# arturxe2/T-DEED

Hardware: AMD Instinct MI355X
Metric: clips/sec (L=100, 224^2, bf16) forward, per-frame logits (higher is better)
Workload: dtype bf16; 1 GPU; rny002_b8: rny002_gsf + ed_sgp_mixer n_layers=2 ks=7, L=100, 224x224, batch 8/GPU, inference forward, random-init weights; clips_per_gpu=8, parallelism=dp1 (clip-sharded, no collective), hip_graph=True, batches_in_flight=3, sub_batches_per_batch=1, dist_backend=none, dist_ranks=1, self_launched=False

## Files before the change

### include/tdeed_hip.h

```cpp
#ifndef TDEED_HIP_H
#define TDEED_HIP_H
#include <stdint.h>
#ifdef __cplusplus
extern "C" {
#endif

enum { TDEED_F32 = 0, TDEED_BF16 = 1 };
enum { TDEED_ACT_NONE = 0, TDEED_ACT_RELU = 1, TDEED_ACT_GELU = 2 };
enum { TDEED_OK = 0, TDEED_ERR_ARG = -1, TDEED_ERR_LAUNCH = -2, TDEED_ERR_RUNTIME = -3 };

const char* tdeed_last_error(void);
int tdeed_abi_version(void);
int tdeed_device_info(int dev, char* name64, int* n_cu, int* is_gfx950);

int tdeed_stem_fwd(const void* frames , int frames_f32,
                   int N, int H, int W, int crop_top, int crop_left,
                   int crop_h, int crop_w, int flip ,
                   const unsigned char* flip_mask ,
                   const float* w ,
                   const float* scale , const float* shift , void* out,
                   int relu , int dtype, void* stream);

int tdeed_stem_mfma_parts(int crop_h, int crop_w);
int tdeed_stem_mfma_fwd(const void* frames, int frames_f32, int N, int H, int W, int crop_top, int crop_left, int crop_h,
// ... 43 lines not shown
int tdeed_gemm_splitk_fwd(const void* A, long lda, int M, int K, int N, const void* W, long ldw, const float* scale,
                          const float* shift, const void* R, long ldr, int act, void* C, long ldc,
                          float* workspace, void* stream);

int tdeed_se_gate_mfma_fits(int C, int R);
int tdeed_se_gate_mfma_fwd(const float* pooled, int n_parts, float inv_cnt, int N, int C, int R, const void* w1f,
                           const float* b1, const void* w2f, const float* b2, float* gate, void* stream);

int tdeed_gemm_rs_fits(int M, int K, int N);
int tdeed_gemm_rs_fwd(const void* A, long lda, const void* A0, long lda0, int k0, const float* a_scale, int a_scale_rows,
                      int M, int K, int N, const void* Wfrag, const float* scale, const float* shift, const void* R, long ldr,
                      int act, void* C, long ldc, void* C2, long ldc2, int n2, void* stream);

int tdeed_gemm_rs_grid(int M);
int tdeed_gemm_rs_stats_fwd(const void* A, long lda, const void* A0, long lda0, int k0, int M, int K, int N, const void* Wfrag,
                            void* C, long ldc, float* colpart, void* stream);

int tdeed_c1_gconv_set_debug(void* buf);
int tdeed_c1_gconv_fits(int Hi, int Wi, int Cin, int C, int stride);
int tdeed_c1_gconv_slab_tiles(int Hi, int Wi, int C, int stride);
int tdeed_c1_gconv_fwd(const void* x, const void* G, int Fp, int N, int Hi, int Wi, int Cin, int C, int gw, int stride,
                       const void* w1f, const float* s1, const float* h1, const void* wfrag, const float* scale,
                       const float* shift, void* y, float* pooled, void* stream);

int tdeed_bneck_fits(int h, int w, int C, int R);
int tdeed_bneck_set_debug(void* buf);
int tdeed_bneck_fwd(const void* x, const void* G, int Fp, int N, int h, int w, int C, const void* w1f, const float* s1,
                    const float* h1, const void* w2f, const float* s2, const float* h2, const void* se_w1f,
                    const float* se_b1, const void* se_w2f, const float* se_b2, int R, const void* w3f, const float* s3,
                    const float* h3, void* out, void* out2, int n2,
                    int w2_tap_major ,
                    void* stream);
int tdeed_bneck_qtail_fits(int h, int w, int C, int F);
int tdeed_bneck_gs_fwd(const void* x, const void* gx, int ldx, const float* gate, const float* ysum, const float* xsum,
                       const float* cw1, const float* cb1, const float* cw2, const float* cb2, int T, int F, int Fp, int N,
                       int h, int w, int C, const void* w1f, const float* s1, const float* h1, const void* w2f,
                       const float* s2, const float* h2, const void* se_w1f, const float* se_b1, const void* se_w2f,
                       const float* se_b2, int R, const void* w3f, const float* s3, const float* h3, void* out, void* out2,
                       int n2, int w2_tap_major, const void* q_wqf, const float* q_bn, int q_F, float* Q, void* stream);


int tdeed_se_gate_fwd(const float* pooled, int n_parts, float inv_cnt, int N, int C, int R,
                      const float* w1t, const float* b1, const float* w2t, const float* b2,
                      float* gate, void* stream);

int tdeed_se_gate_bf16_fwd(const float* pooled, int n_parts, float inv_cnt, int N, int C, int R,
// ... 278 lines not shown
```

### t-deed_amd/_lib.py

```python
import ctypes
import os
from ctypes import c_int, c_long, c_float, c_double, c_void_p, c_char_p, c_uint64, POINTER

import torch

CSRC = os.path.join(os.path.dirname(os.path.abspath(__file__)), "csrc")
LIB_PATH = os.path.join(CSRC, "libtdeed_hip.so")

F32, BF16 = 0, 1
ACT_NONE, ACT_RELU, ACT_GELU = 0, 1, 2


class HipLibraryMissing(RuntimeError):
    pass


class HipCallError(RuntimeError):
    pass


P = c_void_p
_SIGS = {
    "tdeed_abi_version": ([], c_int),
    "tdeed_device_info": ([c_int, c_char_p, POINTER(c_int), POINTER(c_int)], c_int),
# ... 15 lines not shown
    "tdeed_gemm_ws_fits": ([c_int, c_int, c_int], c_int),
    "tdeed_gemm_ws_fwd": ([P, c_long, P, c_long, c_int, P, c_int, c_int, c_int, c_int, P, P, P, P, c_long,
                           c_int, P, c_long, c_int, c_int, c_int, c_int, c_int, P, c_long, c_int, c_int, P], c_int),
    "tdeed_gemm_ws_sc_fits": ([c_int, c_int, c_int, c_int], c_int),
    "tdeed_gemm_ws_sc_fwd": ([P, c_long, P, c_long, c_int, P, c_int, c_int, c_int, c_int, P, P, P, P, c_long, c_int, P, P, P,
                              c_int, P, c_long, c_int, c_int, c_int, c_int, c_int, P, c_long, c_int, c_int, P], c_int),
    "tdeed_gconv3x3_parts": ([c_int, c_int, c_int, c_int, c_int], c_int),
    "tdeed_gconv3x3_mfma_fits": ([c_int, c_int, c_int, c_int], c_int),
    "tdeed_gconv3x3_fwd": ([P, c_int, c_int, c_int, c_int, c_int, c_int, P, P, P, P, P, P, P, P, P, c_int, c_int, P], c_int),
    "tdeed_gemm_splitk_splits": ([c_int], c_int),
    "tdeed_gemm_splitk_fwd": ([P, c_long, c_int, c_int, c_int, P, c_long, P, P, P, c_long, c_int, P, c_long, P, P], c_int),
    "tdeed_se_gate_mfma_fits": ([c_int, c_int], c_int),
    "tdeed_se_gate_mfma_fwd": ([P, c_int, c_float, c_int, c_int, c_int, P, P, P, P, P, P], c_int),
    "tdeed_gemm_rs_fits": ([c_int, c_int, c_int], c_int),
    "tdeed_gemm_rs_grid": ([c_int], c_int),
    "tdeed_gemm_rs_stats_fwd": ([P, c_long, P, c_long, c_int, c_int, c_int, c_int, P, P, c_long, P, P], c_int),
    "tdeed_gemm_rs_fwd": ([P, c_long, P, c_long, c_int, P, c_int, c_int, c_int, c_int, P, P, P, P, c_long, c_int, P, c_long, P,
                           c_long, c_int, P], c_int),
    "tdeed_c1_gconv_set_debug": ([P], c_int),
    "tdeed_c1_gconv_fits": ([c_int, c_int, c_int, c_int, c_int], c_int),
    "tdeed_c1_gconv_slab_tiles": ([c_int, c_int, c_int, c_int], c_int),
    "tdeed_c1_gconv_fwd": ([P, P, c_int, c_int, c_int, c_int, c_int, c_int, c_int, c_int, P, P, P, P, P, P, P, P,
                            P], c_int),
    "tdeed_bneck_fits": ([c_int, c_int, c_int, c_int], c_int),
    "tdeed_bneck_set_debug": ([P], c_int),
    "tdeed_bneck_fwd": ([P, P, c_int, c_int, c_int, c_int, c_int, P, P, P, P, P, P, P, P, P, P, c_int, P, P, P, P, P, c_int,
                         c_int, P], c_int),
    "tdeed_bneck_gs_fwd": ([P, P, c_int, P, P, P, P, P, P, P, c_int, c_int, c_int, c_int, c_int, c_int, c_int, P, P, P, P, P, P, P,
                            P, P, P, c_int, P, P, P, P, P, c_int, c_int, P, P, c_int, P, P], c_int),
    "tdeed_bneck_qtail_fits": ([c_int, c_int, c_int, c_int], c_int),
    "tdeed_gsf_gate_sums_fwd": ([P, c_int, c_int, c_int, c_int, c_int, c_int, P, P, P, P, P, P], c_int),
    "tdeed_bn_slabs": ([c_long], c_int),
    "tdeed_bn_train_stats": ([P, c_long, c_int, P, P, c_float, c_float, P, P, P, P, P, P, P, c_int, P], c_int),
    "tdeed_bn_apply": ([P, c_long, c_int, P, P, P, c_int, P, c_int, P], c_int),
    "tdeed_bn_apply_slice": ([P, c_long, c_int, P, P, P, P, P, c_int, P, P, c_int, c_int, c_int, P], c_int),
    "tdeed_bn_apply2": ([P, c_long, c_int, P, P, P, P, P, c_int, P, c_int, P], c_int),
    "tdeed_bn_train_bwd": ([P, P, P, c_int, c_long, c_int, P, P, P, P, P, P, P, P, P, P, P, c_int, P], c_int),
    "tdeed_fold_rows": ([P, c_long, c_int, c_int, c_int, P, c_long, P], c_int),
    "tdeed_bn_finalize": ([P, P, c_long, c_int, c_long, c_int, P, P, c_float, c_float, P, P, P, P, P, P, P], c_int),
    "tdeed_pool_rows": ([P, P, c_int, c_int, c_int, P, P, c_int, P, c_int, P], c_int),
    "tdeed_se_train_fwd": ([P, c_int, c_int, c_int, P, P, P, P, P, P, P], c_int),
    "tdeed_se_train_bwd": ([P, P, P, c_int, c_int, c_int, P, P, P, P, P, P], c_int),
    "tdeed_scale_rows": ([P, P, P, c_float, c_int, c_int, c_int, P, P, P, c_int, P], c_int),
    "tdeed_gconv3x3_dgrad_stats": ([P, c_int, c_int, c_int, c_int, c_int, P, P, P, P, P, P, P, P, P, P, P], c_int),
    "tdeed_gconv3x3_bwd_stats_bands": ([c_int], c_int),
    "tdeed_gconv3x3_bwd_stats_fits": ([c_int, c_int, c_int, c_int, c_int], c_int),
# ... 211 lines not shown
```

### t-deed_amd/csrc/conv.hip

```cpp
#include "common.h"

template <typename T, typename IN>
__global__ __launch_bounds__(256) void stem_kernel(const IN* __restrict__ frames, int H, int W,
                                                   int top, int left, int ch, int cw, int flip_all,
                                                   const unsigned char* __restrict__ flip_mask,
                                                   const float* __restrict__ w,
                                                   const float* __restrict__ scale,
                                                   const float* __restrict__ shift, T* __restrict__ out,
                                                   int Ho, int Wo, int relu) {
  __shared__ float tile[3][33][34];
  const int n = blockIdx.z;
  const int oy0 = blockIdx.y * 16, ox0 = blockIdx.x * 16;
  const int iy0 = oy0 * 2 - 1, ix0 = ox0 * 2 - 1;
  const float mean[3] = {0.485f, 0.456f, 0.406f};
  const float stdv[3] = {0.229f, 0.224f, 0.225f};
  const IN* src = frames + (long)n * 3 * H * W;
  const int flip = flip_mask ? (int)flip_mask[n] : flip_all;
  for (int i = threadIdx.x; i < 3 * 33 * 33; i += 256) {
    int c = i / (33 * 33);
    int r = i - c * 33 * 33;
    int y = r / 33, x = r - y * 33;
    int iy = iy0 + y, ix = ix0 + x;
    float v = 0.f;
    if (iy >= 0 && iy < ch && ix >= 0 && ix < cw) {
// ... 504 lines not shown
    TD_ISSUE_FENCE();
#pragma unroll
    for (int b8 = 0; b8 < 8; ++b8) {
      const int i = i0 + b8 * 256;
      if (i < total) {
        int j, pix;
        dcpp.divmod(i, pix, j);
        if constexpr (AFF) {
          const bf16x8 t8 = *reinterpret_cast<const bf16x8*>(&v[b8]);
          bf16x8 o8;
#pragma unroll
          for (int e = 0; e < 8; ++e) o8[e] = (bf16_t)fmaxf(fmaf((float)t8[e], ia[e], ib[e]), 0.f);
          v[b8] = *reinterpret_cast<const u32x4*>(&o8);
        }
        *reinterpret_cast<u32x4*>(tile + (long)pix * PS + j * 16) = ok[b8] ? v[b8] : (u32x4){0u, 0u, 0u, 0u};
      }
    }
  }
  __syncthreads();
  gconv_band_mma<STRIDE>(gw_, tile, red, redq, Wi, C, wfrag, scale, shift, y, pooled, pooled_sq, Ho, Wo, nbands, CSP, PS, relu, n, bnd,
                         slab, oy0, nrows_out, bst);
}

template <int STRIDE, int KS1>
__global__ __launch_bounds__(256, KS1 == 4 ? 3 : 1) void c1_gconv_mfma_kernel(const bf16_t* __restrict__ x, const bf16_t* __restrict__ G, int Fp,
                                                            int Hi, int Wi, int Cin, int C, const bf16x8* __restrict__ w1f,
                                                            const float* __restrict__ s1, const float* __restrict__ h1,
                                                            const bf16x8* __restrict__ wfrag, const float* __restrict__ scale,
                                                            const float* __restrict__ shift, bf16_t* __restrict__ y,
                                                            float* __restrict__ pooled, int Ho, int Wo, int band, int nbands,
                                                            int CSP, int PS, int rows_in, int relu, long long* dbg) {
  extern __shared__ __attribute__((aligned(16))) unsigned char tile[];
  __shared__ float red[4][32];
  __shared__ float redq[4][32];
  GC_STAMP(0);
  const long lid = xcd_logical_id(blockIdx.x, gridDim.x);
  const int nslabs_ = (C + CSP - 1) >> (CSP == 64 ? 6 : (CSP == 32 ? 5 : 4));
  int slab, bnd, n, t_;
  td_split(lid, nslabs_, t_, slab);
  td_split(t_, nbands, n, bnd);
  const int oy0 = bnd * band;
  const int nrows_out = min(band, Ho - oy0);
  const int WP = Wi + 2;
  const int iy0 = oy0 * STRIDE - 1;
  const int nrow_used = (nrows_out - 1) * STRIDE + 3;
  const int tid = threadIdx.x, lane = tid & 63, wv = __builtin_amdgcn_readfirstlane(tid >> 6);
  const int pl = lane & 15, q = lane >> 4;
  const int nts = CSP >> 4;
  GcW gw_;
  if constexpr (KS1 <= 2) gw_ = gconv_load_w(wfrag, slab, CSP);
  bf16x8 w1r[4][KS1];
  float a1[4][4], b1[4][4];
#pragma unroll
  for (int t = 0; t < 4; ++t) {
    const int tt = slab * nts + min(t, nts - 1);
#pragma unroll
    for (int ks = 0; ks < KS1; ++ks) w1r[t][ks] = w1f[((long)tt * KS1 + ks) * 64 + lane];
    const int c4 = slab * CSP + t * 16 + 4 * q;
    const bool ok = t < nts && c4 < C;
    const int cc4 = min(c4, C - 4);
    const f32x4 av = *reinterpret_cast<const f32x4*>(s1 + cc4), bv = *reinterpret_cast<const f32x4*>(h1 + cc4);
#pragma unroll
    for (int e = 0; e < 4; ++e) {
      a1[t][e] = ok ? av[e] : 0.f;
      b1[t][e] = ok ? bv[e] : 0.f;
    }
  }
  {
    const int cpp = PS >> 4;
    for (int i = tid; i < nrow_used * 2 * cpp; i += 256) {
      const int j = i % cpp, rc = i / cpp;
      const int rr = rc >> 1, col = (rc & 1) ? (Wi + 1) : 0;
      *reinterpret_cast<u32x4*>(tile + ((long)rr * WP + col) * PS + j * 16) = (u32x4){0u, 0u, 0u, 0u};
// ... 39 lines not shown
#pragma unroll
            for (int ks = 0; ks < KS1; ++ks) acc = __builtin_amdgcn_mfma_f32_16x16x32_bf16(w1r[t][ks], xfi[ks], acc, 0, 0, 0);
            if (pok_) {
              bf16x4 o;
#pragma unroll
              for (int e = 0; e < 4; ++e) o[e] = (bf16_t)fmaxf(acc[e] * a1[t][e] + b1[t][e], 0.f);
              *reinterpret_cast<bf16x4*>(dst + t * 32) = o;
            }
          }
        }
      };
      bf16x8 xa[KS1], xb[KS1];
      int ra, ca, rb, cb;
      bool pa = tile_px(wv, ra, ca), pb;
      tile_load(ra, ca, xa);
      for (int tb = wv; tb < ntl; tb += 8) {
        pb = tile_px(tb + 4, rb, cb);
        tile_load(rb, cb, xb);
        tile_mma(pa, ra, ca, xa);
        pa = tile_px(tb + 8, ra, ca);
        tile_load(ra, ca, xa);
        tile_mma(pb, rb, cb, xb);
      }
    } else
    for (int tb = wv; tb < ntl; tb += 4 * NPF) {
      bf16x8 xf[NPF][KS1];
      int rrs[NPF], ccs[NPF];
      bool poks[NPF];
#pragma unroll
      for (int g = 0; g < NPF; ++g) {
        const int t0 = tb + 4 * g;
        const int p = t0 * 16 + pl;
        poks[g] = t0 < ntl && p < npx;
        dwi.divmod(poks[g] ? p : 0, rrs[g], ccs[g]);
        const long pix = (long)(r_lo + rrs[g]) * Wi + ccs[g];
#pragma unroll
        for (int ks = 0; ks < KS1; ++ks) {
          const int k = 32 * ks + 8 * q;
          const bool ok = poks[g] && k < Cin;
          const bf16_t* src = (gn && k < Fp) ? gn + pix * Fp + k : xn + pix * Cin + k;
          const u32x4 v = *reinterpret_cast<const u32x4*>(ok ? src : xn);
          const u32x4 z = {0u, 0u, 0u, 0u};
          const u32x4 w = ok ? v : z;
          xf[g][ks] = *reinterpret_cast<const bf16x8*>(&w);
        }
      }
#pragma unroll
      for (int g = 0; g < NPF; ++g) {
        if (tb + 4 * g >= ntl) break;
        const bool pok = poks[g];
        unsigned char* dst = tile + ((long)(r_lo + rrs[g] - iy0) * WP + ccs[g] + 1) * PS + 8 * q;
#pragma unroll
        for (int t = 0; t < 4; ++t) {
          if (t < nts) {
            f32x4 acc = {0.f, 0.f, 0.f, 0.f};
#pragma unroll
            for (int ks = 0; ks < KS1; ++ks) acc = __builtin_amdgcn_mfma_f32_16x16x32_bf16(w1r[t][ks], xf[g][ks], acc, 0, 0, 0);
            if (pok) {
              bf16x4 o;
#pragma unroll
              for (int e = 0; e < 4; ++e) o[e] = (bf16_t)fmaxf(acc[e] * a1[t][e] + b1[t][e], 0.f);
              *reinterpret_cast<bf16x4*>(dst + t * 32) = o;
            }
          }
        }
      }
    }
  }
  GC_STAMP(2);
  if constexpr (KS1 > 2) gw_ = gconv_load_w(wfrag, slab, CSP);
  __syncthreads();
  GC_STAMP(3);
  gconv_band_mma<STRIDE>(gw_, tile, red, redq, Wi, C, wfrag, scale, shift, y, pooled, nullptr, Ho, Wo, nbands, CSP, PS, relu, n, bnd,
                         slab, oy0, nrows_out, GcStat{nullptr, nullptr, nullptr, nullptr}, dbg);
}

static long long* g_c1g_dbg = nullptr;
extern "C" int tdeed_c1_gconv_set_debug(void* buf) { g_c1g_dbg = (long long*)buf; return TDEED_OK; }

extern "C" int tdeed_gconv3x3_mfma_fits(int Hi, int Wi, int C, int stride) {
  return gc_geom(Hi, Wi, C, stride).band > 0 ? 1 : 0;
}

extern "C" int tdeed_gconv3x3_parts(int Hi, int Wi, int C, int stride, int dtype) {
  if (dtype != TDEED_BF16) return 1;
  GcGeom g = gc_geom(Hi, Wi, C, stride);
  return g.band > 0 ? g.nbands : 1;
}

static int gconv3x3_launch(const void* x, int N, int Hi, int Wi, int C, int gw, int stride, const float* w, const void* wfrag,
                           const float* scale, const float* shift, void* y, float* pooled, float* pooled_sq, const float* in_a,
                           const float* in_b, int relu, int dtype, void* stream, const GcStat bst);
extern "C" int tdeed_gconv3x3_fwd(const void* x, int N, int Hi, int Wi, int C, int gw, int stride,
// ... 59 lines not shown
}
extern "C" int tdeed_c1_gconv_slab_tiles(int Hi, int Wi, int C, int stride) {
  const GcGeom g = gc_geom(Hi, Wi, C, stride);
  return g.nslabs * (g.CSP >> 4);
}
extern "C" int tdeed_c1_gconv_fwd(const void* x, const void* G, int Fp, int N, int Hi, int Wi, int Cin, int C, int gw,
                                  int stride, const void* w1f, const float* s1, const float* h1, const void* wfrag,
                                  const float* scale, const float* shift, void* y, float* pooled, void* stream) {
  TD_CHECK(x && w1f && s1 && h1 && wfrag && scale && shift && y && pooled, "c1_gconv: null pointer");
  TD_CHECK((gw == 8 || gw == 16) && C % gw == 0, "c1_gconv: group width %d / C %d unsupported", gw, C);
  TD_CHECK(stride == 1 || stride == 2, "c1_gconv: stride %d", stride);
  TD_CHECK(N > 0 && N <= 65535 && tdeed_c1_gconv_fits(Hi, Wi, Cin, C, stride), "c1_gconv: Hi=%d Wi=%d Cin=%d C=%d unsupported",
           Hi, Wi, Cin, C);
  TD_CHECK(!G || (Fp % 8 == 0 && Fp > 0 && Fp <= Cin), "c1_gconv: bad splice width %d", Fp);
  const GcGeom g = gc_geom(Hi, Wi, C, stride);
  const int Ho = (Hi - 1) / stride + 1, Wo = (Wi - 1) / stride + 1;
  dim3 grid((unsigned)((long)g.nbands * g.nslabs * N));
  const size_t smem = (size_t)g.rows_in * (Wi + 2) * g.PS;
  hipStream_t st = (hipStream_t)stream;
  const int KS1 = (Cin + 31) / 32;
#define TD_C1G(Sv, Kv)                                                                                                     \
  hipLaunchKernelGGL((c1_gconv_mfma_kernel<Sv, Kv>), grid, dim3(256), smem, st, (const bf16_t*)x, (const bf16_t*)G,           \
                     G ? Fp : 0, Hi, Wi, Cin, C, (const bf16x8*)w1f, s1, h1, (const bf16x8*)wfrag, scale, shift, (bf16_t*)y,  \
                     pooled, Ho, Wo, g.band, g.nbands, g.CSP, g.PS, g.rows_in, 1, g_c1g_dbg)
#define TD_C1G_K(Sv)                                                                                                       \
  do {                                                                                                                     \
    if (KS1 == 1) TD_C1G(Sv, 1); else if (KS1 == 2) TD_C1G(Sv, 2); else if (KS1 == 4) TD_C1G(Sv, 4);                      \
    else TD_C1G(Sv, 5);                                                                                                    \
  } while (0)
  if (stride == 2) TD_C1G_K(2); else TD_C1G_K(1);
#undef TD_C1G_K
#undef TD_C1G
  TD_LAUNCH_CHECK("c1_gconv");
  return TDEED_OK;
}

#define SE_FPB 4
__global__ __launch_bounds__(256) void se_gate_kernel(const float* __restrict__ pooled, int n_parts, float inv_cnt,
                                                      int N, int C, int R, const float* __restrict__ w1t,
                                                      const float* __restrict__ b1,
                                                      const float* __restrict__ w2t,
                                                      const float* __restrict__ b2, float* __restrict__ gate) {
  extern __shared__ float sm[];
  float* sp = sm;
  float* shid = sm + SE_FPB * C;
  const int f0 = blockIdx.x * SE_FPB;
  for (int i = threadIdx.x; i < SE_FPB * C; i += 256) {
    const int f = i / C, c = i - f * C;
    float v = 0.f;
    if (f0 + f < N) {
      const float* src = pooled + ((long)(f0 + f) * n_parts) * C + c;
      for (int q = 0; q < n_parts; ++q) v += src[(long)q * C];
    }
    sp[i] = v * inv_cnt;
  }
  __syncthreads();
// ... 508 lines not shown
```

### t-deed_amd/engine.py

```python
import os
from collections import namedtuple
from types import SimpleNamespace

import numpy as np
import torch

from . import ops, _lib
from .streams import new_stream
from .regnet_spec import regnet_spec, sgp_up_size, pyramid_lengths, first_site_block
from .packing import (_np, _f32, _dense, pack_ws_weights, pack_se_bf16, pack_mfma_frags, pack_se_mfma,
                      pack_front_weights, _stem_frags_np, gs_source_order_columns, _gsf_q_frags_np, pack_gsf_q_frags,
                      _gsf_p_frags_np, pack_gsf_p_frags, pack_gconv_frags, _gconv_frags_np, stem_frags_on_device,
                      gsf_q_frags_on_device, gconv_frag_index, gconv_frags_on_device)

BN_EPS = 1e-5


class _Pool:

    def __init__(self, device):
        self.device = device
        self.free = []
        self.all = []

# ... 114 lines not shown
    o.up = _np(sd[pre + ".convkw1.weight"]).shape[-1]
    o.w_cat = _dense(_np(sd[pre + ".concat_fc.weight"]).reshape(C, 6 * C), act_dtype, device)
    o.b_cat = _f32(_np(sd[pre + ".concat_fc.bias"]), device)
    o.wcg = (pack_mfma_frags(_np(sd[pre + ".concat_fc.weight"]).reshape(C, 6 * C), device, ks_mult=12)
             if act_dtype == torch.bfloat16 and str(device) != "cpu" and C % 16 == 0 and SGP_GEMM else None)
    _pack_mlp(sd, pre, C, o, act_dtype, device)
    return o


def _se(pooled, inv_cnt, bw, gate):
    if bw.se_mf is not None:
        return ops.se_gate_mfma(pooled, inv_cnt, bw.se_mf.w1f, bw.se_b1, bw.se_mf.w2f, bw.se_b2, bw.spec.se_rd, out=gate)
    if bw.se_bf is not None:
        return ops.se_gate_bf16(pooled, inv_cnt, bw.se_bf.se_w1p, bw.se_b1, bw.se_bf.se_w2p, bw.se_b2, bw.spec.se_rd, out=gate)
    return ops.se_gate(pooled, inv_cnt, bw.se_w1t, bw.se_b1, bw.se_w2t, bw.se_b2, out=gate)


BNECK_ONE_LAUNCH = os.environ.get("TDEED_BNECK", "1") == "1"
BNECK_BLEND = True
BNECK_QTAIL = True
C1_GCONV = os.environ.get("TDEED_C1_GCONV", "1") == "1"
C1_GCONV_MAX_CIN = 160
SC_IN_CONV3 = True


BlockForm = namedtuple("BlockForm", "h w h2 w2 one_launch c1g site Fp slice_in q_given blend_in qtail slice_next sc_in_conv3")


def block_forms(blocks, h, w, act_dtype, taps, last_out_is_slice):
    forms = []
    for bi, bw in enumerate(blocks):
        blk = bw.spec
        nbw = blocks[bi + 1] if bi + 1 < len(blocks) else None
        one_launch = bool(BNECK_ONE_LAUNCH and getattr(bw, "fused", None) is not None and bw.se_mf is not None
                          and blk.stride == 1 and not blk.has_downsample and blk.cin == blk.cout
                          and not (last_out_is_slice and nbw is None) and ops.bneck_fits(h, w, blk.cout, blk.se_rd))
        c1g = bool(C1_GCONV and not one_launch and act_dtype == torch.bfloat16 and bw.w2frag is not None
                   and blk.cin <= C1_GCONV_MAX_CIN and ops.c1_gconv_fits(h, w, blk.cin, blk.cout, blk.stride))
        site = blk.gsf_fold > 0
        Fp = (blk.gsf_fold + 7) // 8 * 8 if site else 0
        blend_in = bool(site and one_launch and BNECK_BLEND and bw.gs_src and bw.gs_cw1 is not None and h * w >= 14
                        and 2 * Fp <= blk.cin and ("_features." + blk.name + ".gs_out") not in taps)
        slice_next = (nbw.spec.gsf_fold + 7) // 8 * 8 if (nbw is not None and nbw.spec.gsf_fold) else 0
        qtail = bool(blend_in and BNECK_QTAIL and slice_next and getattr(nbw, "gs_wqf", None) is not None
                     and ops.bneck_qtail_fits(h, w, blk.cout, nbw.spec.gsf_fold))
        sc_in_conv3 = bool(SC_IN_CONV3 and blk.has_downsample and act_dtype == torch.bfloat16 and bw.w3.ws and bw.wd.ws
                           and ops.gemm_ws_sc_fits(blk.cout, blk.cin, blk.cout, act_dtype))
        h2, w2 = (h - 1) // blk.stride + 1, (w - 1) // blk.stride + 1
        slice_in, q_given = bool(site and forms and forms[-1].slice_next == Fp), bool(forms and forms[-1].qtail)
        forms.append(BlockForm(h, w, h2, w2, one_launch, c1g, site, Fp, slice_in, q_given, blend_in, qtail, slice_next, sc_in_conv3))
        h, w = h2, w2
    return forms


class Step:
    __slots__ = ("name", "kernel", "fn", "bytes", "flops")

    def __init__(self, name, kernel, fn, nbytes=0, flops=0):
        self.name, self.kernel, self.fn, self.bytes, self.flops = name, kernel, fn, int(nbytes), int(flops)


def _esz(dt):
    return 2 if dt == torch.bfloat16 else 4


def gemm_cost(M, K, N, es, residual=False, extra=0):
    return (M * K + N * K + M * N * (2 if residual else 1)) * es + extra, 2 * M * K * N


class SgpBuilder:

    def __init__(self, pool, steps, keep, taps, B, act_dtype):
        self.pool, self.steps, self.keep, self.taps, self.B, self.dt = pool, steps, keep, taps, B, act_dtype
# ... 413 lines not shown
        o2 = xs_next.view(-1, f.slice_next) if f.slice_next else None
        q_next = None
        if f.blend_in:
            qt = None
            if f.qtail:
                q_next = pool.take((N, f.h, f.w, 6), torch.float32)
                qt = (nbw.gs_wpf, nbw.gs_bnq, nbw.spec.gsf_fold, q_next)
            run = lambda: ops.bneck_gs(
                x, xg, gb["gate"], gb["ysum"], gb["xsum"], bw.gs_cw1, bw.gs_cb1, bw.gs_cw2, bw.gs_cb2, T, blk.gsf_fold, f.Fp,
                bw.fused.w1f, bw.s1, bw.h1, bw.fused.w2f, bw.s2, bw.h2, bw.se_mf.w1f, bw.se_b1, bw.se_mf.w2f, bw.se_b2,
                blk.se_rd, bw.fused.w3f, bw.s3, bw.h3, out=out, out2=o2, w2_tap_major=bw.fused.w2_tap_major, qtail=qt)
        else:
            G = gb.get("out")
            run = lambda: ops.bneck(
                x, bw.fused.w1f, bw.s1, bw.h1, bw.fused.w2f, bw.s2, bw.h2, bw.se_mf.w1f, bw.se_b1, bw.se_mf.w2f, bw.se_b2,
                blk.se_rd, bw.fused.w3f, bw.s3, bw.h3, G=G, out=out, out2=o2, w2_tap_major=bw.fused.w2_tap_major)
        steps.append(Step(blk.name + ".bneck", "bneck", run,
                          (2 * M * blk.cout + (M * f.Fp if f.blend_in else 0)) * es + (8 * M if f.blend_in else 0)
                          + (24 * M if f.qtail else 0)
                          + (2 * blk.cout * blk.cout + blk.cout * blk.gw * 9) * es,
                          2 * M * blk.cout * (2 * blk.cout + blk.gw * 9)))
        return out, xs_next, q_next

    def _chain(self, pool, steps, B, bw, f, x, y1, G, out, dead_site):
        blk, dt = bw.spec, self.act_dtype
        N, es, s = B * self.pw.clip_len, _esz(dt), blk.stride
        h, w, h2, w2 = f.h, f.w, f.h2, f.w2
        M, M2 = N * h * w, N * h2 * w2
        if y1 is not None:
            splice = dict(A0=G, k0=f.Fp) if f.site else {}
            steps.append(Step(blk.name + ".conv1", bw.w1.kern(M), lambda: bw.w1.run(
                x, bw.s1, bw.h1, ops.ACT_RELU, out=y1, M=M, **splice), *gemm_cost(M, blk.cin, blk.cout, es)))
        y2 = pool.take((N, h2, w2, blk.cout), dt)
        parts = ops.gconv3x3_parts(h, w, blk.cout, s, dt) if bw.w2frag is not None else 1
        pooled = pool.take((N, parts, blk.cout), torch.float32)
        gate = pool.take((N, blk.cout), torch.float32)
        if f.c1g:
            if bw.c1g_w1f is None:
                bw.c1g_w1f = pack_mfma_frags(bw.w1_raw, self.device, rows=16 * ops.c1_gconv_slab_tiles(h, w, blk.cout, s))
            steps.append(Step(blk.name + ".conv1_conv2", "c1_gconv", lambda: ops.c1_gconv(
                x, bw.c1g_w1f, bw.s1, bw.h1, bw.w2frag, bw.s2, bw.h2, blk.gw, s, blk.cout, G=G, out=y2, pooled=pooled),
                (M * blk.cin + M2 * blk.cout) * es + blk.cout * (blk.cin + blk.gw * 9) * es,
                2 * M * blk.cin * blk.cout + 2 * M2 * blk.cout * blk.gw * 9))
        else:
            steps.append(Step(blk.name + ".conv2", "gconv3x3", lambda: ops.gconv3x3(
                y1, bw.w2, bw.s2, bw.h2, blk.gw, s, wfrag=bw.w2frag, out=y2, pooled=pooled),
                (M + M2) * blk.cout * es + blk.cout * blk.gw * 9 * 4, 2 * M2 * blk.cout * blk.gw * 9))
        sc, shortcut, sc_from = x, [], None
        gather = (s, h, w, h2, w2) if s > 1 else None
        if f.sc_in_conv3:
            sc, sc_from = None, (x, gather)
        elif blk.has_downsample:
            sc = pool.take((N, h2, w2, blk.cout), dt)
            shortcut = [Step(blk.name + ".downsample", bw.wd.kern(M2), lambda: bw.wd.run(
                x, bw.sd, bw.hd, ops.ACT_NONE, gather=gather, out=sc, M=M2), *gemm_cost(M2, blk.cin, blk.cout, es))]
        if out is None:
            out = pool.take((N, h2, w2, blk.cout), dt)
        xs_next = pool.take((N, h2, w2, f.slice_next), dt) if f.slice_next else None
        se, conv3 = self._se_conv3(bw, N, h2, w2, y2, pooled, gate, sc, out, out2=xs_next, sc_from=sc_from)
        steps += [se, *shortcut, conv3]
        return out, xs_next, ([y1] if y1 is not None else []) + [y2, pooled, gate] + dead_site + ([sc] if shortcut else [])

    def _blocks(self, pool, steps, keep, taps, B, x, h, w, blocks, x_kept, out_last=None):
        N, dt = B * self.pw.clip_len, self.act_dtype
        xs = q = None
        for bi, f in enumerate(block_forms(blocks, h, w, dt, taps, out_last is not None)):
            bw, last = blocks[bi], bi + 1 == len(blocks)
            y1 = None if (f.one_launch or f.c1g) else pool.take((N, f.h, f.w, bw.spec.cout), dt)
            xg = xs if f.slice_in else x
            gb = self._gs_site(pool, steps, keep, taps, B, bw, f, xg, q) if f.site else {}
            dead = list(gb.values()) + ([xs] if f.slice_in else [])
            if f.one_launch:
                out, xs, q = self._one_launch(pool, steps, B, bw, f, x, xg, gb, None if last else blocks[bi + 1])
            else:
                out, xs, dead = self._chain(pool, steps, B, bw, f, x, y1, gb.get("out"), out_last if last else None, dead)
                q = None
            x_kept = self._block_done(pool, keep, taps, bw.spec, dead, x, x_kept, out)
            x, h, w = out, f.h2, f.w2
        return x, h, w, x_kept

    def _build_tail(self, B, feat, head_out, trunk_in=None, start=None):
        pool, steps, keep = _Pool(self.device), [], {}
        if trunk_in is not None:
            x, h, w = trunk_in
            x, h, w, _ = self._blocks(pool, steps, keep, set(), B, x, h, w, list(self.pw.W.blocks[start:]), True)
            self._avgpool(steps, B, x, h, w, feat)
        cur = self._sgp_heads(pool, steps, keep, set(), B, feat, head_out)
        return SimpleNamespace(steps=steps, pool_bytes=pool.total_bytes(), sgp_out=cur)

    def _build(self, B, H, W, flip, taps, head_out=None, feat_out=None, stop_at=None, trunk_out=None, feat_rs=None,
               frames_dtype=torch.uint8):
        pw, Wt = self.pw, self.pw.W
        T = pw.clip_len
        N = B * T
        dt = self.act_dtype
        dev = self.device
        pool = _Pool(dev)
        steps = []
        keep = {}
        crop = None
        ch, cw = H, W
        if self.crop_dim is not None and self.crop_dim > 0 and (self.crop_dim != H or self.crop_dim != W):
            ch = cw = self.crop_dim
            crop = (int(round((H - ch) / 2.0)), int(round((W - cw) / 2.0)), ch, cw)
        frames = torch.empty((N, 3, H, W), dtype=frames_dtype, device=dev)
        Ho, Wo = (ch + 1) // 2, (cw + 1) // 2
        es = _esz(dt)
        blocks = list(Wt.blocks)
        fused_front = (Wt.front is not None and "_features.stem" not in taps and self.fuse_front
                       and frames_dtype == torch.uint8 and not isinstance(flip, torch.Tensor)
                       and ops.s1_front_parts(ch, cw, Wt.blocks[0].spec.cout) > 0)
        if fused_front:
            bw = blocks.pop(0)
            blk = bw.spec
            h2, w2 = (Ho + 1) // 2, (Wo + 1) // 2
            parts = ops.s1_front_parts(ch, cw, blk.cout)
            y2 = pool.take((N, h2, w2, blk.cout), dt)
            sc = pool.take((N, h2, w2, blk.cout), dt)
            pooled = pool.take((N, parts, blk.cout), torch.float32)
            gate = pool.take((N, blk.cout), torch.float32)
            out = pool.take((N, h2, w2, blk.cout), dt)
            M2 = N * h2 * w2
            steps.append(Step("s1_front", "s1_front", lambda y2=y2, sc=sc, pooled=pooled: ops.s1_front(
                frames, Wt.front, crop, flip, y2=y2, shortcut=sc, pooled=pooled),
                              N * 3 * ch * cw + 2 * M2 * blk.cout * es,
                              2 * N * Ho * Wo * 32 * (27 + 2 * blk.cout) // 1 + 2 * M2 * blk.cout * blk.gw * 9))
            steps += self._se_conv3(bw, N, h2, w2, y2, pooled, gate, sc, out)
            x_kept = self._block_done(pool, keep, taps, blk, (y2, sc, pooled, gate), None, True, out)
            x, h, w = out, h2, w2
        else:
            x = pool.take((N, Ho, Wo, 32), dt)
            steps.append(Step("stem", "stem", lambda x=x: ops.stem(frames, Wt.stem_w, Wt.stem_scale, Wt.stem_shift, dt, crop,
                                                                   flip, out=x),
                              N * 3 * ch * cw + N * Ho * Wo * 32 * es, 2 * N * Ho * Wo * 32 * 27))
            h, w = Ho, Wo
            x_kept = "_features.stem" in taps
            if x_kept:
                keep["_features.stem"] = x
        if stop_at is not None:
            blocks = blocks[:max(0, stop_at - (1 if fused_front else 0))]
        if trunk_out is not None and not blocks:
            raise ValueError("join_at must leave at least one un-fused bottleneck in the sub-batch plans")
        x, h, w, x_kept = self._blocks(pool, steps, keep, taps, B, x, h, w, blocks, x_kept, out_last=trunk_out)
        if stop_at is not None:
            return SimpleNamespace(frames=frames, steps=steps, keep=keep, head_out=None, pool_bytes=pool.total_bytes(), B=B, T=T,
                                   h=h, w=w)
        feat = pool.take((B, T, pw.spec.feat_dim), sgp_stream_dtype(dt, dev)) if feat_out is None else feat_out
        self._avgpool(steps, B, x, h, w, feat, feat_rs)
        keep["feat"] = feat
        if not x_kept:
            pool.give(x)
        if feat_out is not None:
            return SimpleNamespace(frames=frames, steps=steps, keep=keep, head_out=None, pool_bytes=pool.total_bytes(), B=B, T=T)

        if head_out is None:
            head_out = torch.empty((N, pw.n_out), dtype=torch.float32, device=dev)
        keep["sgp_out"] = self._sgp_heads(pool, steps, keep, taps, B, feat, head_out)
        return SimpleNamespace(frames=frames, steps=steps, keep=keep, head_out=head_out,
                               pool_bytes=pool.total_bytes(), B=B, T=T)

    def _map_geometry(self, k, H, W):
        ch = self.crop_dim if (self.crop_dim and self.crop_dim > 0) else H
        cw = self.crop_dim if (self.crop_dim and self.crop_dim > 0) else W
        hh, ww = (ch + 1) // 2, (cw + 1) // 2
        for b_ in self.pw.W.blocks[:k]:
            hh, ww = (hh - 1) // b_.spec.stride + 1, (ww - 1) // b_.spec.stride + 1
# ... 250 lines not shown
```

### t-deed_amd/ops.py

```python
import ctypes

import torch

from . import _lib
from ._lib import call, ptr, stream_ptr, dtype_code, ACT_NONE, ACT_RELU, ACT_GELU


def _chk(t, name, dtype=None):
    if t is None:
        return
    if not t.is_cuda:
        raise RuntimeError(f"{name} must be a GPU tensor (tdeed_amd has no CPU path)")
    if not t.is_contiguous():
        raise RuntimeError(f"{name} must be contiguous")
    if dtype is not None and t.dtype != dtype:
        raise TypeError(f"{name}: expected {dtype}, got {t.dtype}")


def _flip_args(flip, N):
    if isinstance(flip, torch.Tensor):
        m = flip.to(torch.uint8).contiguous()
        if m.numel() != N or not m.is_cuda:
            raise ValueError(f"flip mask must hold one flag per frame on the GPU ({m.numel()} vs {N})")
        return 0, m
# ... 89 lines not shown
         ptr(residual), (residual.shape[-1] if residual is not None else 0), act, ptr(out), ldc,
         g[0], g[1], g[2], g[3], g[4], ptr(colpart), *_out2(out2, A), int(bool(out2_pre)), dtype_code(A.dtype), stream_ptr())
    return out


def c1_gconv_fits(Hi, Wi, Cin, C, stride):
    return _lib.load().tdeed_c1_gconv_fits(Hi, Wi, Cin, C, stride) != 0


def c1_gconv_slab_tiles(Hi, Wi, C, stride):
    return _lib.load().tdeed_c1_gconv_slab_tiles(Hi, Wi, C, stride)


def c1_gconv(x, w1f, s1, h1, wfrag, scale, shift, gw, stride, C, G=None, out=None, pooled=None):
    _chk(x, "x", torch.bfloat16); _chk(G, "G", torch.bfloat16)
    N, Hi, Wi, Cin = x.shape
    Ho, Wo = (Hi - 1) // stride + 1, (Wi - 1) // stride + 1
    if out is None:
        out = torch.empty((N, Ho, Wo, C), dtype=x.dtype, device=x.device)
    if pooled is None:
        pooled = torch.empty((N, gconv3x3_parts(Hi, Wi, C, stride, x.dtype), C), dtype=torch.float32, device=x.device)
    call("tdeed_c1_gconv_fwd", ptr(x), ptr(G), (G.shape[-1] if G is not None else 0), N, Hi, Wi, Cin, C, gw, stride, ptr(w1f),
         ptr(s1), ptr(h1), ptr(wfrag), ptr(scale), ptr(shift), ptr(out), ptr(pooled), stream_ptr())
    return out, pooled


def bneck_fits(h, w, C, R):
    return _lib.load().tdeed_bneck_fits(h, w, C, R) != 0


def bneck(x, w1f, s1, h1, w2f, s2, h2, se_w1f, se_b1, se_w2f, se_b2, R, w3f, s3, h3, G=None, out=None, out2=None,
          w2_tap_major=True):
    _chk(x, "x", torch.bfloat16); _chk(G, "G", torch.bfloat16); _chk(out2, "out2", torch.bfloat16)
    N, h, w, C = x.shape
    if out is None:
        out = torch.empty_like(x)
    call("tdeed_bneck_fwd", ptr(x), ptr(G), (G.shape[-1] if G is not None else 0), N, h, w, C, ptr(w1f), ptr(s1),
         ptr(h1), ptr(w2f), ptr(s2), ptr(h2), ptr(se_w1f), ptr(se_b1), ptr(se_w2f), ptr(se_b2), R, ptr(w3f), ptr(s3), ptr(h3),
         ptr(out), ptr(out2), (out2.shape[-1] if out2 is not None else 0), int(bool(w2_tap_major)), stream_ptr())
    return out


def bneck_gs(x, gx, gate, ysum, xsum, cw1, cb1, cw2, cb2, T, F, Fp, w1f, s1, h1, w2f, s2, h2, se_w1f, se_b1, se_w2f, se_b2, R,
             w3f, s3, h3, out=None, out2=None, w2_tap_major=True, qtail=None):
    _chk(x, "x", torch.bfloat16); _chk(gx, "gx", torch.bfloat16); _chk(out2, "out2", torch.bfloat16)
    N, h, w, C = x.shape
# ... 830 lines not shown
```

Before: 5506 clips/s.

## Fuse stage-1 front conv3 epilogue into next block's conv1+gconv kernel

Adds a C3IN variant of the c1_gconv kernel. It computes the preceding front block's SE-gated conv3, BN, residual add and ReLU inline, then feeds that result straight into conv1 and the grouped 3x3 conv. This removes the separate conv3 launch and the full-resolution write and read of the front block's output. Only the stride-2 subsampled copy is stored for the shortcut path. The cost is more per-pixel work and loads inside the gconv kernel (both y2 and the shortcut tensor), a changed occupancy hint, and extra plumbing in block planning.

```diff
diff --git a/include/tdeed_hip.h b/include/tdeed_hip.h
--- a/include/tdeed_hip.h
+++ b/include/tdeed_hip.h
@@ -89,6 +89,12 @@
 int tdeed_c1_gconv_fwd(const void* x, const void* G, int Fp, int N, int Hi, int Wi, int Cin, int C, int gw, int stride,
                        const void* w1f, const float* s1, const float* h1, const void* wfrag, const float* scale,
                        const float* shift, void* y, float* pooled, void* stream);
+
+int tdeed_c1_gconv_c3in_fits(int Hi, int Wi, int Cp, int C);
+int tdeed_c1_gconv_c3in_fwd(const void* y2p, const void* scp, const float* gate, const void* w3f, const float* s3,
+                            const float* h3, void* xs2, int N, int Hi, int Wi, int Cp, int C, int gw, const void* w1f,
+                            const float* s1, const float* h1, const void* wfrag, const float* scale, const float* shift,
+                            void* y, float* pooled, void* stream);
 
 int tdeed_bneck_fits(int h, int w, int C, int R);
 int tdeed_bneck_set_debug(void* buf);
diff --git a/t-deed_amd/_lib.py b/t-deed_amd/_lib.py
--- a/t-deed_amd/_lib.py
+++ b/t-deed_amd/_lib.py
@@ -61,6 +61,9 @@
     "tdeed_c1_gconv_slab_tiles": ([c_int, c_int, c_int, c_int], c_int),
     "tdeed_c1_gconv_fwd": ([P, P, c_int, c_int, c_int, c_int, c_int, c_int, c_int, c_int, P, P, P, P, P, P, P, P,
                             P], c_int),
+    "tdeed_c1_gconv_c3in_fits": ([c_int, c_int, c_int, c_int], c_int),
+    "tdeed_c1_gconv_c3in_fwd": ([P, P, P, P, P, P, P, c_int, c_int, c_int, c_int, c_int, c_int, P, P, P, P, P, P, P, P,
+                                 P], c_int),
     "tdeed_bneck_fits": ([c_int, c_int, c_int, c_int], c_int),
     "tdeed_bneck_set_debug": ([P], c_int),
     "tdeed_bneck_fwd": ([P, P, c_int, c_int, c_int, c_int, c_int, P, P, P, P, P, P, P, P, P, P, c_int, P, P, P, P, P, c_int,
diff --git a/t-deed_amd/csrc/conv.hip b/t-deed_amd/csrc/conv.hip
--- a/t-deed_amd/csrc/conv.hip
+++ b/t-deed_amd/csrc/conv.hip
@@ -550,14 +550,21 @@
                          slab, oy0, nrows_out, bst);
 }
 
-template <int STRIDE, int KS1>
-__global__ __launch_bounds__(256, KS1 == 4 ? 3 : 1) void c1_gconv_mfma_kernel(const bf16_t* __restrict__ x, const bf16_t* __restrict__ G, int Fp,
+struct C3In {
+  const bf16_t* y2p; const bf16_t* scp; const float* gate;
+  const bf16x8* w3f; const float* s3; const float* h3;
+  bf16_t* xs2;
+};
+template <int STRIDE, int KS1, bool C3IN = false>
+__global__ __launch_bounds__(256, (KS1 == 4 || C3IN) ? 3 : 1) void c1_gconv_mfma_kernel(const bf16_t* __restrict__ x, const bf16_t* __restrict__ G, int Fp,
                                                             int Hi, int Wi, int Cin, int C, const bf16x8* __restrict__ w1f,
                                                             const float* __restrict__ s1, const float* __restrict__ h1,
                                                             const bf16x8* __restrict__ wfrag, const float* __restrict__ scale,
                                                             const float* __restrict__ shift, bf16_t* __restrict__ y,
                                                             float* __restrict__ pooled, int Ho, int Wo, int band, int nbands,
-                                                            int CSP, int PS, int rows_in, int relu, long long* dbg) {
+                                                            int CSP, int PS, int rows_in, int relu, long long* dbg,
+                                                            const C3In c3) {
+  static_assert(!C3IN || (STRIDE == 2 && KS1 == 1), "the conv3-in-front form exists for stride 2 and one k-step");
   extern __shared__ __attribute__((aligned(16))) unsigned char tile[];
   __shared__ float red[4][32];
   __shared__ float redq[4][32];
@@ -575,8 +582,9 @@
   const int tid = threadIdx.x, lane = tid & 63, wv = __builtin_amdgcn_readfirstlane(tid >> 6);
   const int pl = lane & 15, q = lane >> 4;
   const int nts = CSP >> 4;
+  constexpr bool GW_EARLY = KS1 <= 2 && !C3IN;
   GcW gw_;
-  if constexpr (KS1 <= 2) gw_ = gconv_load_w(wfrag, slab, CSP);
+  if constexpr (GW_EARLY) gw_ = gconv_load_w(wfrag, slab, CSP);
   bf16x8 w1r[4][KS1];
   float a1[4][4], b1[4][4];
 #pragma unroll
@@ -662,6 +670,90 @@
         tile_load(ra, ca, xa);
         tile_mma(pb, rb, cb, xb);
       }
+    } else if constexpr (C3IN) {
+      const int k8 = 8 * q;
+      const bool kok = k8 < Cin;
+      const int kc = min(k8, Cin - 8);
+      const bf16_t* yn = c3.y2p + (long)n * Hi * Wi * Cin;
+      const bf16_t* rn = c3.scp + (long)n * Hi * Wi * Cin;
+      const bf16x8 w3a = c3.w3f[lane], w3b = c3.w3f[64 + lane];
+      float g8[8], sc3[8], sh3[8];
+#pragma unroll
+      for (int e4 = 0; e4 < 8; e4 += 4) {
+        const f32x4 gv = *reinterpret_cast<const f32x4*>(c3.gate + (long)n * Cin + kc + e4);
+        const f32x4 sv = *reinterpret_cast<const f32x4*>(c3.s3 + kc + e4), hv = *reinterpret_cast<const f32x4*>(c3.h3 + kc + e4);
+#pragma unroll
+        for (int e = 0; e < 4; ++e) {
+          g8[e4 + e] = gv[e];
+          sc3[e4 + e] = kok ? sv[e] : 1.f;
+          sh3[e4 + e] = kok ? hv[e] : 0.f;
+        }
+      }
+      bf16_t* xsn = c3.xs2 ? c3.xs2 + (long)n * Ho * Wo * Cin : nullptr;
+      for (int tb = wv; tb < ntl; tb += 4 * NPF) {
+        u32x4 yf[NPF], rf[NPF];
+        int rrs[NPF], ccs[NPF];
+        bool poks[NPF];
+#pragma unroll
+        for (int g = 0; g < NPF; ++g) {
+          const int t0 = tb + 4 * g;
+          const int p = t0 * 16 + pl;
+          poks[g] = t0 < ntl && p < npx;
+          dwi.divmod(poks[g] ? p : 0, rrs[g], ccs[g]);
+          const long o = ((long)(r_lo + rrs[g]) * Wi + ccs[g]) * Cin + kc;
+          yf[g] = *reinterpret_cast<const u32x4*>(yn + o);
+          rf[g] = *reinterpret_cast<const u32x4*>(rn + o);
+        }
+#pragma unroll
+        for (int g = 0; g < NPF; ++g) {
+          if (tb + 4 * g >= ntl) break;
+          const bool pok = poks[g];
+          const bf16x8 y8 = *reinterpret_cast<const bf16x8*>(&yf[g]), r8 = *reinterpret_cast<const bf16x8*>(&rf[g]);
+          bf16x8 a8;
+#pragma unroll
+          for (int e = 0; e < 8; ++e) {
+            float f = (float)y8[e];
+            f *= g8[e];
+            a8[e] = (bf16_t)f;
+          }
+          const u32x4 zero4 = {0u, 0u, 0u, 0u};
+          const u32x4 am = (pok && kok) ? *reinterpret_cast<const u32x4*>(&a8) : zero4;
+          const f32x4 z4 = {0.f, 0.f, 0.f, 0.f};
+          const f32x4 c0 = __builtin_amdgcn_mfma_f32_16x16x32_bf16(w3a, *reinterpret_cast<const bf16x8*>(&am), z4, 0, 0, 0);
+          const f32x4 c1 = __builtin_amdgcn_mfma_f32_16x16x32_bf16(w3b, *reinterpret_cast<const bf16x8*>(&am), z4, 0, 0, 0);
+          float v[8];
+#pragma unroll
+          for (int r = 0; r < 4; ++r) {
+            v[r] = c0[r] * sc3[r] + sh3[r];
+            v[4 + r] = c1[r] * sc3[4 + r] + sh3[4 + r];
+          }
+          bf16x8 o8;
+#pragma unroll
+          for (int e = 0; e < 8; ++e) {
+            v[e] += (float)r8[e];
+            v[e] = fmaxf(v[e], 0.f);
+            o8[e] = (bf16_t)v[e];
+          }
+          const u32x4 xm = kok ? *reinterpret_cast<const u32x4*>(&o8) : zero4;
+          const bf16x8 xf = *reinterpret_cast<const bf16x8*>(&xm);
+          const int row = r_lo + rrs[g], col = ccs[g];
+          if (xsn && pok && kok && !((row | col) & 1) && (row >> 1) >= oy0 && (row >> 1) < oy0 + nrows_out)
+            *reinterpret_cast<u32x4*>(xsn + ((long)(row >> 1) * Wo + (col >> 1)) * Cin + k8) = xm;
+          unsigned char* dst = tile + ((long)(row - iy0) * WP + col + 1) * PS + 8 * q;
+#pragma unroll
+          for (int t = 0; t < 4; ++t) {
+            if (t < nts) {
+              const f32x4 acc = __builtin_amdgcn_mfma_f32_16x16x32_bf16(w1r[t][0], xf, z4, 0, 0, 0);
+              if (pok) {
+                bf16x4 o;
+#pragma unroll
+                for (int e = 0; e < 4; ++e) o[e] = (bf16_t)fmaxf(acc[e] * a1[t][e] + b1[t][e], 0.f);
+                *reinterpret_cast<bf16x4*>(dst + t * 32) = o;
+              }
+            }
+          }
+        }
+      }
     } else
     for (int tb = wv; tb < ntl; tb += 4 * NPF) {
       bf16x8 xf[NPF][KS1];
@@ -708,7 +800,7 @@
     }
   }
   GC_STAMP(2);
-  if constexpr (KS1 > 2) gw_ = gconv_load_w(wfrag, slab, CSP);
+  if constexpr (!GW_EARLY) gw_ = gconv_load_w(wfrag, slab, CSP);
   __syncthreads();
   GC_STAMP(3);
   gconv_band_mma<STRIDE>(gw_, tile, red, redq, Wi, C, wfrag, scale, shift, y, pooled, nullptr, Ho, Wo, nbands, CSP, PS, relu, n, bnd,
@@ -814,7 +906,7 @@
 #define TD_C1G(Sv, Kv)                                                                                                     \
   hipLaunchKernelGGL((c1_gconv_mfma_kernel<Sv, Kv>), grid, dim3(256), smem, st, (const bf16_t*)x, (const bf16_t*)G,           \
                      G ? Fp : 0, Hi, Wi, Cin, C, (const bf16x8*)w1f, s1, h1, (const bf16x8*)wfrag, scale, shift, (bf16_t*)y,  \
-                     pooled, Ho, Wo, g.band, g.nbands, g.CSP, g.PS, g.rows_in, 1, g_c1g_dbg)
+                     pooled, Ho, Wo, g.band, g.nbands, g.CSP, g.PS, g.rows_in, 1, g_c1g_dbg, C3In{})
 #define TD_C1G_K(Sv)                                                                                                       \
   do {                                                                                                                     \
     if (KS1 == 1) TD_C1G(Sv, 1); else if (KS1 == 2) TD_C1G(Sv, 2); else if (KS1 == 4) TD_C1G(Sv, 4);                      \
@@ -824,6 +916,31 @@
 #undef TD_C1G_K
 #undef TD_C1G
   TD_LAUNCH_CHECK("c1_gconv");
+  return TDEED_OK;
+}
+
+extern "C" int tdeed_c1_gconv_c3in_fits(int Hi, int Wi, int Cp, int C) {
+  if (Cp < 8 || Cp > 32 || Cp % 8 != 0 || C > 64 || !tdeed_c1_gconv_fits(Hi, Wi, Cp, C, 2)) return 0;
+  return gc_geom(Hi, Wi, C, 2).nslabs == 1 ? 1 : 0;
+}
+extern "C" int tdeed_c1_gconv_c3in_fwd(const void* y2p, const void* scp, const float* gate, const void* w3f, const float* s3,
+                                       const float* h3, void* xs2, int N, int Hi, int Wi, int Cp, int C, int gw,
+                                       const void* w1f, const float* s1, const float* h1, const void* wfrag,
+                                       const float* scale, const float* shift, void* y, float* pooled, void* stream) {
+  TD_CHECK(y2p && scp && gate && w3f && s3 && h3, "c1_gconv_c3in: null pointer (the producer's operands)");
+  TD_CHECK(w1f && s1 && h1 && wfrag && scale && shift && y && pooled, "c1_gconv_c3in: null pointer");
+  TD_CHECK((gw == 8 || gw == 16) && C % gw == 0, "c1_gconv_c3in: group width %d / C %d unsupported", gw, C);
+  TD_CHECK(N > 0 && N <= 65535 && tdeed_c1_gconv_c3in_fits(Hi, Wi, Cp, C), "c1_gconv_c3in: Hi=%d Wi=%d Cp=%d C=%d unsupported",
+           Hi, Wi, Cp, C);
+  const GcGeom g = gc_geom(Hi, Wi, C, 2);
+  const int Ho = (Hi - 1) / 2 + 1, Wo = (Wi - 1) / 2 + 1;
+  dim3 grid((unsigned)((long)g.nbands * N));
+  const size_t smem = (size_t)g.rows_in * (Wi + 2) * g.PS;
+  const C3In c3{(const bf16_t*)y2p, (const bf16_t*)scp, gate, (const bf16x8*)w3f, s3, h3, (bf16_t*)xs2};
+  hipLaunchKernelGGL((c1_gconv_mfma_kernel<2, 1, true>), grid, dim3(256), smem, (hipStream_t)stream, (const bf16_t*)nullptr,
+                     (const bf16_t*)nullptr, 0, Hi, Wi, Cp, C, (const bf16x8*)w1f, s1, h1, (const bf16x8*)wfrag, scale, shift,
+                     (bf16_t*)y, pooled, Ho, Wo, g.band, g.nbands, g.CSP, g.PS, g.rows_in, 1, g_c1g_dbg, c3);
+  TD_LAUNCH_CHECK("c1_gconv_c3in");
   return TDEED_OK;
 }
 
diff --git a/t-deed_amd/engine.py b/t-deed_amd/engine.py
--- a/t-deed_amd/engine.py
+++ b/t-deed_amd/engine.py
@@ -160,12 +160,14 @@
 C1_GCONV = os.environ.get("TDEED_C1_GCONV", "1") == "1"
 C1_GCONV_MAX_CIN = 160
 SC_IN_CONV3 = True
-
-
-BlockForm = namedtuple("BlockForm", "h w h2 w2 one_launch c1g site Fp slice_in q_given blend_in qtail slice_next sc_in_conv3")
-
-
-def block_forms(blocks, h, w, act_dtype, taps, last_out_is_slice):
+S1_CONV3_IN_C1G = True
+
+
+BlockForm = namedtuple("BlockForm",
+                       "h w h2 w2 one_launch c1g site Fp slice_in q_given blend_in qtail slice_next sc_in_conv3 conv3_in")
+
+
+def block_forms(blocks, h, w, act_dtype, taps, last_out_is_slice, pending=None):
     forms = []
     for bi, bw in enumerate(blocks):
         blk = bw.spec
@@ -186,7 +188,12 @@
                            and ops.gemm_ws_sc_fits(blk.cout, blk.cin, blk.cout, act_dtype))
         h2, w2 = (h - 1) // blk.stride + 1, (w - 1) // blk.stride + 1
         slice_in, q_given = bool(site and forms and forms[-1].slice_next == Fp), bool(forms and forms[-1].qtail)
-        forms.append(BlockForm(h, w, h2, w2, one_launch, c1g, site, Fp, slice_in, q_given, blend_in, qtail, slice_next, sc_in_conv3))
+        conv3_in = bool(S1_CONV3_IN_C1G and pending is not None and bi == 0 and c1g and not site and blk.stride == 2
+                        and blk.has_downsample and act_dtype == torch.bfloat16 and pending.w3.ws
+                        and pending.spec.cout == blk.cin and ("_features." + pending.spec.name) not in taps
+                        and ops.c1_gconv_c3in_fits(h, w, blk.cin, blk.cout))
+        forms.append(BlockForm(h, w, h2, w2, one_launch, c1g, site, Fp, slice_in, q_given, blend_in, qtail, slice_next, sc_in_conv3,
+                               conv3_in))
         h, w = h2, w2
     return forms
 
@@ -646,7 +653,7 @@
                           2 * M * blk.cout * (2 * blk.cout + blk.gw * 9)))
         return out, xs_next, q_next
 
-    def _chain(self, pool, steps, B, bw, f, x, y1, G, out, dead_site):
+    def _chain(self, pool, steps, B, bw, f, x, y1, G, out, dead_site, front=None):
         blk, dt = bw.spec, self.act_dtype
         N, es, s = B * self.pw.clip_len, _esz(dt), blk.stride
         h, w, h2, w2 = f.h, f.w, f.h2, f.w2
@@ -659,9 +666,21 @@
         parts = ops.gconv3x3_parts(h, w, blk.cout, s, dt) if bw.w2frag is not None else 1
         pooled = pool.take((N, parts, blk.cout), torch.float32)
         gate = pool.take((N, blk.cout), torch.float32)
-        if f.c1g:
-            if bw.c1g_w1f is None:
-                bw.c1g_w1f = pack_mfma_frags(bw.w1_raw, self.device, rows=16 * ops.c1_gconv_slab_tiles(h, w, blk.cout, s))
+        if f.c1g and bw.c1g_w1f is None:
+            bw.c1g_w1f = pack_mfma_frags(bw.w1_raw, self.device, rows=16 * ops.c1_gconv_slab_tiles(h, w, blk.cout, s))
+        xs2 = None
+        if f.conv3_in:
+            pbw = front.bw
+            xs2 = pool.take((N, h2, w2, blk.cin), dt)
+            steps.append(Step(blk.name + ".conv1_conv2", "c1_gconv", lambda: ops.c1_gconv_c3in(
+                front.y2, front.sc, front.gate, pbw.w3.w, pbw.s3, pbw.h3, bw.c1g_w1f, bw.s1, bw.h1, bw.w2frag, bw.s2, bw.h2,
+                blk.gw, blk.cout, xs2=xs2, out=y2, pooled=pooled),
+                (2 * M * blk.cin + M2 * blk.cout + M2 * blk.cin) * es + (blk.cin * blk.cin + blk.cout * (blk.cin + blk.gw * 9)) * es,
+                2 * M * blk.cin * blk.cin + 2 * M * blk.cin * blk.cout + 2 * M2 * blk.cout * blk.gw * 9))
+            for t_ in (front.y2, front.sc, front.pooled, front.gate):
+                pool.give(t_)
+            x = xs2
+        elif f.c1g:
             steps.append(Step(blk.name + ".conv1_conv2", "c1_gconv", lambda: ops.c1_gconv(
                 x, bw.c1g_w1f, bw.s1, bw.h1, bw.w2frag, bw.s2, bw.h2, blk.gw, s, blk.cout, G=G, out=y2, pooled=pooled),
                 (M * blk.cin + M2 * blk.cout) * es + blk.cout * (blk.cin + blk.gw * 9) * es,
@@ -671,7 +690,7 @@
                 y1, bw.w2, bw.s2, bw.h2, blk.gw, s, wfrag=bw.w2frag, out=y2, pooled=pooled),
                 (M + M2) * blk.cout * es + blk.cout * blk.gw * 9 * 4, 2 * M2 * blk.cout * blk.gw * 9))
         sc, shortcut, sc_from = x, [], None
-        gather = (s, h, w, h2, w2) if s > 1 else None
+        gather = (s, h, w, h2, w2) if (s > 1 and xs2 is None) else None
         if f.sc_in_conv3:
             sc, sc_from = None, (x, gather)
         elif blk.has_downsample:
@@ -683,12 +702,23 @@
         xs_next = pool.take((N, h2, w2, f.slice_next), dt) if f.slice_next else None
         se, conv3 = self._se_conv3(bw, N, h2, w2, y2, pooled, gate, sc, out, out2=xs_next, sc_from=sc_from)
         steps += [se, *shortcut, conv3]
-        return out, xs_next, ([y1] if y1 is not None else []) + [y2, pooled, gate] + dead_site + ([sc] if shortcut else [])
-
-    def _blocks(self, pool, steps, keep, taps, B, x, h, w, blocks, x_kept, out_last=None):
+        return out, xs_next, (([y1] if y1 is not None else []) + [y2, pooled, gate] + dead_site + ([sc] if shortcut else [])
+                              + ([xs2] if xs2 is not None else []))
+
+    def _blocks(self, pool, steps, keep, taps, B, x, h, w, blocks, x_kept, out_last=None, front=None):
         N, dt = B * self.pw.clip_len, self.act_dtype
         xs = q = None
-        for bi, f in enumerate(block_forms(blocks, h, w, dt, taps, out_last is not None)):
+        forms = block_forms(blocks, h, w, dt, taps, out_last is not None, *(() if front is None else (front.bw,)))
+        if front is not None:
+            if forms and forms[0].conv3_in:
+                steps.append(self._se_conv3(front.bw, N, h, w, front.y2, front.pooled, front.gate, front.sc, None)[0])
+            else:
+                x = pool.take((N, h, w, front.bw.spec.cout), dt)
+                steps += self._se_conv3(front.bw, N, h, w, front.y2, front.pooled, front.gate, front.sc, x)
+                x_kept = self._block_done(pool, keep, taps, front.bw.spec, (front.y2, front.sc, front.pooled, front.gate), None,
+                                          True, x)
+                front = None
+        for bi, f in enumerate(forms):
             bw, last = blocks[bi], bi + 1 == len(blocks)
             y1 = None if (f.one_launch or f.c1g) else pool.take((N, f.h, f.w, bw.spec.cout), dt)
             xg = xs if f.slice_in else x
@@ -697,7 +727,8 @@
             if f.one_launch:
                 out, xs, q = self._one_launch(pool, steps, B, bw, f, x, xg, gb, None if last else blocks[bi + 1])
             else:
-                out, xs, dead = self._chain(pool, steps, B, bw, f, x, y1, gb.get("out"), out_last if last else None, dead)
+                out, xs, dead = self._chain(pool, steps, B, bw, f, x, y1, gb.get("out"), out_last if last else None, dead,
+                                            front if f.conv3_in else None)
                 q = None
             x_kept = self._block_done(pool, keep, taps, bw.spec, dead, x, x_kept, out)
             x, h, w = out, f.h2, f.w2
@@ -743,16 +774,15 @@
             sc = pool.take((N, h2, w2, blk.cout), dt)
             pooled = pool.take((N, parts, blk.cout), torch.float32)
             gate = pool.take((N, blk.cout), torch.float32)
-            out = pool.take((N, h2, w2, blk.cout), dt)
             M2 = N * h2 * w2
             steps.append(Step("s1_front", "s1_front", lambda y2=y2, sc=sc, pooled=pooled: ops.s1_front(
                 frames, Wt.front, crop, flip, y2=y2, shortcut=sc, pooled=pooled),
                               N * 3 * ch * cw + 2 * M2 * blk.cout * es,
                               2 * N * Ho * Wo * 32 * (27 + 2 * blk.cout) // 1 + 2 * M2 * blk.cout * blk.gw * 9))
-            steps += self._se_conv3(bw, N, h2, w2, y2, pooled, gate, sc, out)
-            x_kept = self._block_done(pool, keep, taps, blk, (y2, sc, pooled, gate), None, True, out)
-            x, h, w = out, h2, w2
+            front = SimpleNamespace(bw=bw, y2=y2, sc=sc, pooled=pooled, gate=gate)
+            x, h, w, x_kept = None, h2, w2, True
         else:
+            front = None
             x = pool.take((N, Ho, Wo, 32), dt)
             steps.append(Step("stem", "stem", lambda x=x: ops.stem(frames, Wt.stem_w, Wt.stem_scale, Wt.stem_shift, dt, crop,
                                                                    flip, out=x),
@@ -765,7 +795,7 @@
             blocks = blocks[:max(0, stop_at - (1 if fused_front else 0))]
         if trunk_out is not None and not blocks:
             raise ValueError("join_at must leave at least one un-fused bottleneck in the sub-batch plans")
-        x, h, w, x_kept = self._blocks(pool, steps, keep, taps, B, x, h, w, blocks, x_kept, out_last=trunk_out)
+        x, h, w, x_kept = self._blocks(pool, steps, keep, taps, B, x, h, w, blocks, x_kept, out_last=trunk_out, front=front)
         if stop_at is not None:
             return SimpleNamespace(frames=frames, steps=steps, keep=keep, head_out=None, pool_bytes=pool.total_bytes(), B=B, T=T,
                                    h=h, w=w)
diff --git a/t-deed_amd/ops.py b/t-deed_amd/ops.py
--- a/t-deed_amd/ops.py
+++ b/t-deed_amd/ops.py
@@ -135,6 +135,30 @@
         pooled = torch.empty((N, gconv3x3_parts(Hi, Wi, C, stride, x.dtype), C), dtype=torch.float32, device=x.device)
     call("tdeed_c1_gconv_fwd", ptr(x), ptr(G), (G.shape[-1] if G is not None else 0), N, Hi, Wi, Cin, C, gw, stride, ptr(w1f),
          ptr(s1), ptr(h1), ptr(wfrag), ptr(scale), ptr(shift), ptr(out), ptr(pooled), stream_ptr())
+    return out, pooled
+
+
+def c1_gconv_c3in_fits(Hi, Wi, Cp, C):
+    lib = _lib.load()
+    if not hasattr(lib, "tdeed_c1_gconv_c3in_fits"):
+        return False
+    return lib.tdeed_c1_gconv_c3in_fits(Hi, Wi, Cp, C) != 0
+
+
+def c1_gconv_c3in(y2p, scp, gate, w3frag, s3, h3, w1f, s1, h1, wfrag, scale, shift, gw, C, xs2=None, out=None, pooled=None):
+    _chk(y2p, "y2p", torch.bfloat16); _chk(scp, "scp", torch.bfloat16); _chk(gate, "gate", torch.float32)
+    _chk(xs2, "xs2", torch.bfloat16)
+    N, Hi, Wi, Cp = y2p.shape
+    Ho, Wo = (Hi - 1) // 2 + 1, (Wi - 1) // 2 + 1
+    if tuple(scp.shape) != (N, Hi, Wi, Cp) or gate.numel() != N * Cp or (xs2 is not None and xs2.numel() != N * Ho * Wo * Cp):
+        raise ValueError(f"c1_gconv_c3in: y2p {tuple(y2p.shape)}, scp {tuple(scp.shape)}, gate {tuple(gate.shape)}, "
+                         f"xs2 {None if xs2 is None else tuple(xs2.shape)} do not belong together")
+    if out is None:
+        out = torch.empty((N, Ho, Wo, C), dtype=y2p.dtype, device=y2p.device)
+    if pooled is None:
+        pooled = torch.empty((N, gconv3x3_parts(Hi, Wi, C, 2, y2p.dtype), C), dtype=torch.float32, device=y2p.device)
+    call("tdeed_c1_gconv_c3in_fwd", ptr(y2p), ptr(scp), ptr(gate), ptr(w3frag), ptr(s3), ptr(h3), ptr(xs2), N, Hi, Wi, Cp, C, gw,
+         ptr(w1f), ptr(s1), ptr(h1), ptr(wfrag), ptr(scale), ptr(shift), ptr(out), ptr(pooled), stream_ptr())
     return out, pooled
 
 
```

Result: faster. 5718 clips/s, median of 6 (+3.9%).
